# NADOOIT/whisperX

Hardware: AMD Instinct MI355X
Metric: aligned audio-sec/s + word-boundary MAE(ms) vs ref, 1/2/4/8 GPU (higher is better)
Workload: dtype f32; 1 GPU; cfg2: batch=64 x 30 s EN segments, T=1499, V=32, N~U[300,500]; fused HIP align DP (wx_align_dp) on HBM-resident emissions; global_batch=64, seq_len=1499, parallelism=dp1 (per-file sharding, RCCL vocab broadcast)

## Files before the change

### whisperx_amd/csrc/wx_align_dp.h

```cpp
#ifndef WX_ALIGN_DP_H
#define WX_ALIGN_DP_H

#include "wx_dp_config.h"
#include "wx_dp_forward.h"
#include "wx_dp_helpers.h"
#include "wx_dp_prims.h"
#include "wx_dp_tail.h"
#include "wx_dp_timing.h"
#include "wx_dp_walk.h"
#include "wx_wave.h"

namespace wx {

__device__ unsigned split_arrive(uint64_t* c, unsigned epoch, bool lost) {
    uint64_t old = __hip_atomic_load(c, __ATOMIC_RELAXED, __HIP_MEMORY_SCOPE_AGENT);
    while (true) {
        const unsigned cur = ((unsigned)(old >> 32) == epoch) ? (unsigned)old : 0u;
        const unsigned nw = ((cur & 0x7Fu) + 1u) | (cur & 0x80u) | (lost ? 0x80u : 0u);
        const uint64_t nv = ((uint64_t)epoch << 32) | nw;
        if (__hip_atomic_compare_exchange_strong(c, &old, nv, __ATOMIC_RELAXED, __ATOMIC_RELAXED,
                                                 __HIP_MEMORY_SCOPE_AGENT))
            return nw;
    }
}

constexpr int kLatencyLdsFloats = 84 * 1024 / 4;

template <int VS>
struct ColMapLds {
    static constexpr bool kOn = VS == kGatherVS;
    unsigned bm[kOn ? kMaxVocabWords : 1];
    int wpre[kOn ? kMaxVocabWords + 1 : 1];
    int cols[kOn ? kGatherVS : 1];
};

template <int VS>
__device__ __forceinline__ bool prepare_colmap(ColMapLds<VS>& m, ColMap& cm, const int32_t* tok, int N, int blank,
                                               int V) {
    cm.bm = m.bm;
    cm.wpre = m.wpre;
    cm.cols = m.cols;
    cm.n = 0;
    if (!ColMapLds<VS>::kOn) return true;
    cm.n = build_colmap(tok, N, blank, V, m.bm, m.wpre, m.cols);
    return cm.n <= kGatherVS;
}

template <int VS, int W>
constexpr int kCkSlots = (W == 1 || VS == 32) ? 2 * W : W;

constexpr int kSplitWaves = 8;
constexpr int kQ0LdsFrames = 4096;

template <int C, int VS, int W, int H, bool SP = false, int XW = 0>
__device__ __forceinline__ void align_dp_body(const AlignArgs& a) {
    constexpr bool CK = !SP && H == 0 && VS != kGatherVS && W >= 2;
    constexpr bool WT = split_wt<C, VS, SP>();
    constexpr int kLdsFloats = H ? (kLatencyLdsFloats > 4 * kChunk * VS ? kLatencyLdsFloats : 4 * kChunk * VS)
                                 : (CK ? kCkSlots<VS, W> : 2) * kChunk * VS;
    __shared__ float lds[kLdsFloats];
    __shared__ __attribute__((aligned(16))) float c0b[H || (CK && W >= 2) ? 2 * kChunk : 1];
    __shared__ __attribute__((aligned(16))) float xh[W > 1 ? 2 * W * kWave : 1];
    __shared__ unsigned cmask_lds[kMaxLdsFrames / kChunk + 1];
    __shared__ int tsb[3];
    __shared__ int blo_lds;
    __shared__ int colrec_lds[W + H > 1 ? kMaxLdsFrames / kChunk + 1 : 1];
    __shared__ int sbuf_lds[3 * (W + H + XW)];
    __shared__ ColMapLds<VS> cml;
    __shared__ float xg_lds[SP && C == 1 ? 2 * 32 : 1];
    __shared__ float q0_lds[SP && XW > 0 ? kQ0LdsFrames : 1];
    const int P = SP ? a.parts : 1;
    const int part = SP ? ((int)blockIdx.x / kXcdStride) % P : 0;
    const int xslot = (int)blockIdx.x % kXcdStride;
    const int seg = SP ? ((int)blockIdx.x / kXcdStride / P) * kXcdStride +
                             ((a.flags & kArgXcdSpread) ? (xslot - part) & (kXcdStride - 1) : xslot)
                       : (int)blockIdx.x;
    if (SP && seg >= a.S) return;
    const SegDesc d = load_desc(a.em_off, a.tok_off, a.blank_id, seg);
    const int want = (SP || a.parts > 1) ? launch_split_bucket(d.N, a.parts, a.split_id) : bucket_id(d.N, a.mode);
    if (want != (bucket_make(C, W, H ? 1 : 0) | (SP ? kSplitFlag : 0))) return;
    const int lane = (int)threadIdx.x;
    if (d.N <= 0 || d.T <= 0) {
        if (lane == 0 && part == 0) {
            a.t_start[seg] = 0;
            a.status[seg] = 1;
        }
        return;
    }
    ColMap cm;
    const bool slow = !prepare_colmap(cml, cm, a.tok + d.tok0, d.N, d.blank, a.V);
    if (slow && part != 0) return;
    const float* E = a.em + d.row0 * a.V;
    unsigned* bits = a.bits + ((d.row0 >> 5) + seg) * (int64_t)a.bits_stride_cells;
    float* q0 = a.q0 + d.row0;
    float* cn = a.cn + ((d.row0 + kCnPad * (int64_t)seg) & ~(int64_t)3);
    double* c0acc = a.c0acc + ((d.row0 >> 5) + seg);
    WX_STAMP_RT(4);
    WX_STAMP(0);
    Split sp;
    if (SP) {
        sp.p = part;
        sp.P = P;
        sp.lanes = kWave * W * P;
        sp.tag = a.epoch;
        sp.xstride = (kMaxParts - 1) * kHaloCells;
        sp.spin = a.spin;
        uint64_t* xseg = a.xg + ((d.row0 >> 5) + seg) * (int64_t)sp.xstride;
        sp.xin = xseg + (part > 0 ? part - 1 : 0) * kHaloCells;
        sp.xout = xseg + part * kHaloCells;
        sp.xg = xg_lds;
        sp.q0l = (XW > 0 && d.T <= kQ0LdsFrames) ? q0_lds : nullptr;
    }
    if (SP && lane == 0) tsb[2] = 0;
    bool lost = false;
    if (!slow)
        lost = Forward<C, VS, CK ? 2 : 0, W, H != 0, SP, (H > 1 ? 2 : 1)>::run(
            d, E, a.V, a.tok, bits, q0, cn, nullptr, lds, c0b, xh, a.x4 != 0, cm, nullptr, &sp, c0acc);
    WX_STAMP(1);
    if (SP && lost) tsb[2] = 1;
    wait_vm();
    block_fence();
    bool failed = false;
    if (SP && !slow) {
        if (lane == 0) {
            const bool fenced = !WT || (a.flags & kArgFenced);
            if (fenced) {
                __builtin_amdgcn_fence(__ATOMIC_RELEASE, "agent");
                wait_vm();
            }
            const unsigned w = split_arrive(a.arrive + seg, a.epoch, tsb[2] != 0);
            tsb[0] = ((w & 0x7Fu) == (unsigned)P) ? 1 + (int)((w >> 7) & 1u) : 0;
            if (tsb[0]) {
                if (fenced) {
                    __builtin_amdgcn_fence(__ATOMIC_ACQUIRE, "agent");
                    wait_vm();
                }
                __hip_atomic_store(a.arrive + seg, (uint64_t)0, __ATOMIC_RELAXED, __HIP_MEMORY_SCOPE_AGENT);
            }
        }
        __syncthreads();
        if (tsb[0] == 0) {
            WX_STAMP(2);
            WX_STAMP(3);
            WX_STAMP_RT(5);
            return;
        }
        failed = tsb[0] == 2;
        __syncthreads();
    }
    const Layout lay = Layout::make(C, d.N, kWave * W * P);
    if (slow || failed) {
        if (!generic_forward(d.T, d.N, d.blank, E, a.V, a.tok + d.tok0, bits, lay, cn, q0, lds, kLdsFloats)) {
            if (lane == 0) {
                a.t_start[seg] = 0;
                a.status[seg] = slow ? 2 : 3;
            }
            return;
        }
        wait_vm();
        block_fence();
    }
    int32_t* start = a.seg_start + d.tok0;
    WX_T(w0);
    const int nbw = ((d.T - 1) >> 5) + 1;
    const bool lds_walk = d.T <= kMaxLdsFrames;
    const bool q0l_ok = SP && XW > 0 && d.T <= kQ0LdsFrames && !slow && !failed;
    const int K = lds_walk ? max(1, min(W + H + XW, nbw / kSpecMinBlocks)) : 1;
    WX_T(w1);
    WX_TDECL(w2 = 0);
    auto walk_tail = [&](auto& wsrc) {
    int ts = 0, b_lo = -1;
    unsigned* cmask = lds_walk ? cmask_lds : a.cmask + ((d.row0 >> 5) + seg);
    if constexpr (W + H > 1) b_lo = walk_spec(wsrc, d.N, d.T, cn, cmask, lds_walk, K, colrec_lds, sbuf_lds, ts);
    if (lane < kWave) {
        if constexpr (W + H == 1) {
            ts = column_argmax<WT>(cn, d.T);
            b_lo = walk_impl(wsrc, d.N, ts, cmask, lds_walk);
        }
        if (lane == 0) {
            a.t_start[seg] = ts;
            tsb[0] = ts;
        }
        WX_TSET(w2);
        if (!H && b_lo >= 0) {
            wave_fence();
            compact_starts(cmask, b_lo, (ts - 1) >> 5, start);
        }
        if (lane == 0) {
            tsb[1] = b_lo >= 0 ? 1 : 0;
            blo_lds = b_lo;
        }
    } else {
        if (H && !slow && !failed && !q0l_ok) fill_q0(E, a.V, d.T, q0, kWave);
    }
    if constexpr (H != 0) {
        block_fence();
        const int bl = uniform(blo_lds);
        if (bl >= 0) compact_starts_par(cmask, bl, (uniform(tsb[0]) - 1) >> 5, start);
    }
    WX_T(w3);
    WX_TDUMP(lane == 0, 15, w1 - w0, w2 - w1, w3 - w2);
    };
    if constexpr (CK) {
        CkSrc<C, VS> wsrc;
        wsrc.ck = reinterpret_cast<const float*>(bits);
        wsrc.lay = lay;
        wsrc.acc = c0acc;
        wsrc.E = E;
        wsrc.tok = a.tok + d.tok0;
        wsrc.T = d.T;
        wsrc.N = d.N;
        wsrc.V = a.V;
        wsrc.blank = d.blank;
        wsrc.x4 = a.x4 != 0;
        wsrc.slot[0] = lds + uniform((int)threadIdx.x >> 6) * kChunk * VS;
        wsrc.slot[1] = kCkSlots<VS, W> >= 2 * W ? wsrc.slot[0] + W * kChunk * VS : wsrc.slot[0];
        wsrc.junk = xh;
        walk_tail(wsrc);
    } else {
        BitSrc<C, WT> wsrc{bits, lay};
        walk_tail(wsrc);
    }
    wait_vm();
    block_fence();
    const int ts = tsb[0];
    const bool ok = tsb[1] != 0;
    WX_STAMP(2);
    if (lane == 0) a.status[seg] = (ok ? 0 : 1) | (failed ? WX_STATUS_RECOVERED : 0) | (slow ? WX_STATUS_GENERIC : 0);
    if (!ok) return;
    if (d.T + d.N <= kLdsFloats && d.N > 2 * (int)blockDim.x)
        merge_tokens_lds(E, a.V, a.tok + d.tok0, d.N, d.T, ts, q0l_ok ? q0_lds : q0, start, a.seg_end + d.tok0,
                         a.seg_score + d.tok0, lds);
    else
        merge_tokens(E, a.V, a.tok + d.tok0, d.N, ts, q0l_ok ? q0_lds : q0, start, a.seg_end + d.tok0,
                     a.seg_score + d.tok0);
    WX_STAMP(3);
    WX_STAMP_RT(5);
}

template <int C, int VS, int W, int H>
__global__ __launch_bounds__(kWave*(W + H)) __attribute__((amdgpu_waves_per_eu(H || VS == kGatherVS || C > 8 || W == 1 ? 1 : 4, H ? 2 : 8))) void align_dp_kernel(
    AlignArgs a) {
    align_dp_body<C, VS, W, H>(a);
}

template <int C, int VS, int W>
__global__ __launch_bounds__(kWave * kSplitWaves) __attribute__((amdgpu_waves_per_eu(1, 2))) void align_dp_split_kernel(
    AlignArgs a) {
    static_assert(W + 2 <= kSplitWaves && kSplitWaves <= 8, "split workgroup: W DP waves + 2 helpers + walkers");
    align_dp_body<C, VS, W, 2, true, kSplitWaves - W - 2>(a);
}

template <int C, int VS, int W>
__global__ __launch_bounds__(kWave * W) void trellis_kernel(TrellisArgs a) {
    __shared__ float lds[2 * kChunk * VS];
    __shared__ float xh[W > 1 ? 2 * W * kWave : 1];
    __shared__ ColMapLds<VS> cml;
    __shared__ __attribute__((aligned(16))) float rst[W * kWave * C];
    const int seg = blockIdx.x;
    const SegDesc d = load_desc(a.em_off, a.tok_off, a.blank_id, seg);
    if (bucket_id(d.N) != bucket_make(C, W, 0)) return;
    float* tr = a.tr + a.tr_off[seg];
    const int lane = (int)threadIdx.x;
    if (d.N == 0) {
        for (int t = lane; t <= d.T; t += kWave * W) tr[t] = INFINITY;
        return;
    }
    ColMap cm;
    if (!prepare_colmap(cml, cm, a.tok + d.tok0, d.N, d.blank, a.V)) {
        const int64_t n = (int64_t)(d.T + 1) * (d.N + 1);
        for (int64_t i = lane; i < n; i += kWave * W) tr[i] = NAN;
        return;
    }
    const float* E = a.em + d.row0 * a.V;
    Forward<C, VS, 1, W, false>::run(d, E, a.V, a.tok, nullptr, nullptr, nullptr, tr, lds, nullptr, xh, a.x4 != 0,
                                     cm, rst);
}

}

#endif
```

### whisperx_amd/csrc/wx_dp_forward.h

```cpp
#ifndef WX_DP_FORWARD_H
#define WX_DP_FORWARD_H

#include "wx_dp_config.h"
#include "wx_dp_prims.h"
#include "wx_dp_timing.h"
#include "wx_wave.h"

namespace wx {

template <int C>
using cellvec = float __attribute__((ext_vector_type(C)));

template <int VS>
__host__ __device__ constexpr int quad_stride() { return 4 * (VS + 1); }
template <int VS>
__host__ __device__ constexpr int quad_buf_floats() { return 8 * quad_stride<VS>(); }

constexpr int kXSlack = 1;

struct Split {
    int p, P;
    int lanes;
    unsigned tag;
    uint64_t* xin;
    uint64_t* xout;
    int xstride;
    int spin;
    float* xg;
    float* q0l;
};

template <int C, int VS, int MODE, int W, bool H, bool SP = false, int NH = 1>
struct Forward {
    static constexpr int kRowBytes = VS * 4;
    static constexpr int kLanes = kWave * W;
    static constexpr int kBufs = (C == 1 && MODE == 0 && SP && NH == 2 && VS != kGatherVS) ? 5 : (H ? 4 : 2);
    static constexpr bool kPipelined = H || (MODE != 1 && (C <= 6 || (C == 8 && W == 1)));
    static constexpr bool kC0Lds = H || (MODE == 2 && W >= 2);
    using Geo = Geometry<C, (SP ? 2 : W)>;
    static constexpr int kU = kUnroll;
    static_assert(!(H && MODE == 1), "the materialising kernel computes column 0 in wave 0");
    static constexpr bool kReg = C == 1 && MODE == 0 && SP && NH == 2 && VS != kGatherVS;
    static constexpr bool kWT = split_wt<C, VS, SP>();
    static constexpr int kBufFloats = kReg ? quad_buf_floats<VS>() : kChunk * VS;
    static constexpr int kQS = quad_stride<VS>();

    struct State {
        cellvec<C> cur;
        unsigned w[C];
        double acc;
        float col0;
        int t;
        float* rs;
        int jbase;
        int rd[C];
    };

    __device__ __forceinline__ static bool xwait(const uint64_t* xin, int xstride, int q, int l, unsigned tag,
                                                 uint64_t (&xpre)[C], bool& lost, int spin) {
        constexpr int HL = Geometry<C, 2>::HL;
        const unsigned want = tag;
        const uint64_t* gi = xin + (int64_t)q * xstride + min(l, HL - 1) * C;
        bool ok = true;
#pragma unroll
        for (int k = 0; k < C; ++k) ok = ok && (l >= HL || (unsigned)(xpre[k] >> 32) == want);
        const bool first = __all(ok);
        if (!first) {
            for (int it = 0; !lost && !__all(ok) && it < spin; ++it) {
                __builtin_amdgcn_s_sleep(2);
                ok = true;
#pragma unroll
                for (int k = 0; k < C; ++k) {
                    xpre[k] = granule_load(gi + k);
                    ok = ok && (l >= HL || (unsigned)(xpre[k] >> 32) == want);
                }
            }
            __builtin_amdgcn_s_waitcnt(0x0F70);
        }
        lost = lost || !__all(ok);
        return first;
    }

    __device__ __forceinline__ static bool run(const SegDesc& d, const float* __restrict__ E, int V,
                                               const int32_t* __restrict__ tok,
                                               unsigned* __restrict__ bits,
                                               float* __restrict__ q0,
                                               float* __restrict__ cn,
                                               float* __restrict__ tr,
                                               float* lds ,
                                               float* c0b ,
                                               float* xh , bool x4,
                                               const ColMap& cm ,
                                               float* rst = nullptr ,
                                               const Split* sp = nullptr ,
                                               double* c0acc = nullptr ) {
        const int wv = uniform((int)threadIdx.x >> 6);
        const int vw = SP ? sp->p * W + wv : wv;
        const int lanes = SP ? sp->lanes : kLanes;
        const int T = d.T, N = d.N;
        const int nch = (T + kChunk - 1) / kChunk;
        const bool c0prod = MODE == 2 && W >= 2 && wv == 1;
        double c0a = 0.0;
        float c0e = 0.0f;
        const int l0 = lane_id();
        auto c0_load = [&](int qq) { return E[(int64_t)min(qq * kChunk + (l0 & 31), T - 1) * V]; };
        auto c0_make = [&](int qq, float e) {
            float x = l0 >= 32 ? e : 0.0f;
            double a = c0a;
#pragma unroll
            for (int j = 0; j < kChunk; ++j) {
                a += (double)x;
                x = __builtin_bit_cast(float, __builtin_amdgcn_mov_dpp(__builtin_bit_cast(int, x), 0x130 ,
                                                                       0xF, 0xF, true));
            }
            if (l0 == 0) c0acc[qq] = c0a;
            if (l0 < kChunk) c0b[(qq & 1) * kChunk + l0] = col0_value(qq * kChunk + l0, a, T, N);
            c0a = __shfl(a, kChunk);
        };
        if (c0prod && nch > 0) c0_make(0, c0_load(0));
        if (H && wv >= W + NH) {
            float* q0l = SP ? sp->q0l : nullptr;
            const int nxw = (int)(blockDim.x >> 6) - W - NH;
            const int step = kWave * nxw;
            const int l = lane_id();
            int r0 = (wv - W - NH) * kWave;
            float e0 = 0.0f, e1 = 0.0f;
            if (q0l) {
                e0 = E[(int64_t)min(r0 + l, T - 1) * V];
                e1 = E[(int64_t)min(r0 + step + l, T - 1) * V];
            }
            if (kReg) __syncthreads();
            for (int q = 0; q < nch; ++q) {
                __syncthreads();
                if (q0l && r0 < T) {
                    if (r0 + l < T) q0l[r0 + l] = exp_cr(e0);
                    e0 = e1;
                    r0 += step;
                    e1 = E[(int64_t)min(r0 + step + l, T - 1) * V];
                }
            }
            return false;
        }
        if (H && wv >= W) {
            const bool col0 = (!SP || sp->p == 0) && (NH == 1 || wv == W + 1);
            if constexpr (kReg) {
                int t0 = N > 0 ? tok[d.tok0] : 0;
                t0 = (t0 >= 0 && t0 < V) ? t0 : 0;
                return helper_reg(d, E, V, lds, lds + kBufs * kBufFloats, nch, t0, col0, wv == W, x4, sp);
            } else {
                helper(d, E, V, lds, c0b, nch, x4, cm, col0, NH == 1 || wv == W);
            }
            return false;
        }
        const int l = lane_id();
        const Layout L = Layout::make(C, N, lanes);
        if (MODE == 1) {
            if (threadIdx.x == 0) tr[0] = col0_value(0, 0.0, T, N);
            for (int j = (int)threadIdx.x + 1; j <= N; j += kLanes) tr[j] = -INFINITY;
        }
        if ((W > 1 || SP) && vw > 0 && Geo::lane_of(vw, Geo::HL) >= L.G) {
            if (!H && nch > 0) stage_rows<VS, W>(E, V, 0, min(kChunk, T), lds, x4, cm);
            if (kReg) __syncthreads();
            for (int q = 0; q < nch; ++q) {
                wait_vm();
                __syncthreads();
                if (c0prod && q + 1 < nch) c0_make(q + 1, c0_load(q + 1));
                if (!H && q + 1 < nch)
                    stage_rows<VS, W>(E, V, (q + 1) * kChunk, min(kChunk, T - (q + 1) * kChunk),
                                      lds + ((q + 1) % kBufs) * kBufFloats, x4, cm);
            }
            return false;
        }
        const int g = Geo::lane_of(vw, l);
        const bool halo = vw > 0 && l < Geo::HL;
        const bool xpub = SP && wv == W - 1 && sp->p + 1 < sp->P && Geo::lane_of(vw + 1, Geo::HL) < L.G;
        const bool xsub = SP && wv == 0 && sp->p > 0;
        const int f = L.first(g), cnt = L.count(g);
        const bool is_short = g < L.n_short;
        int toff[C];
#pragma unroll
        for (int k = 0; k < C; ++k) {
            const int j = f + k;
            int tk = (k < cnt && j <= N) ? tok[d.tok0 + j - 1] : 0;
            tk = (tk >= 0 && tk < V) ? tk : 0;
            toff[k] = (VS == kGatherVS ? cm.rank(tk) : tk) * 4;
        }
        const int boff = (VS == kGatherVS ? cm.rank(d.blank) : d.blank) * 4;
        int own_w, own_l;
        Geo::owner(L.G - 1, own_w, own_l);
        const bool owner = uniform(own_w) == vw && l == own_l;
        const bool owner_wave = uniform(own_w) == vw;

        State st;
        if (MODE == 1) {
            const int g0 = Geo::lane_of(vw, vw == 0 ? 0 : Geo::HL);
            const int g1 = min(Geo::lane_of(vw, kWave - 1), L.G - 1);
            const int jend = g1 >= g0 ? L.first(g1) + L.count(g1) - 1 : 0;
            st.jbase = g0 < L.G ? L.first(g0) : N + 1;
            const int nown = max(0, jend - st.jbase + 1);
            st.rs = rst + wv * kWave * C;
#pragma unroll
            for (int i = 0; i < C; ++i) {
                const int r = l + kWave * i;
                int gg = 0, kk = 0;
                if (r < nown) L.locate<C>(st.jbase + r - 1, gg, kk);
                st.rd[i] = r < nown ? (gg - Geo::lane_of(vw, 0)) * C + kk : -1;
            }
        }
#pragma unroll
        for (int k = 0; k < C; ++k) st.cur[k] = -INFINITY;
#pragma unroll
        for (int k = 0; k < C; ++k) st.w[k] = 0u;
        st.acc = 0.0;
        st.col0 = col0_value(0, 0.0, T, N);
        st.t = 0;
        const int inf_from = T + 1 - N;

        if (!H && nch > 0) stage_rows<VS, W>(E, V, 0, min(kChunk, T), lds, x4, cm);
        uint64_t xodd[C], xeven[C];
        bool xlost = false;
#pragma unroll
        for (int k = 0; k < C; ++k) xodd[k] = xeven[k] = 0;
        const int xl = min(l, Geo::HL - 1) * C;
        if (SP && xsub && !kReg) {
#pragma unroll
            for (int k = 0; k < C; ++k) {
                xodd[k] = granule_load(sp->xin + (int64_t)min(1, nch - 1) * sp->xstride + xl + k);
                xeven[k] = granule_load(sp->xin + (int64_t)min(2, nch - 1) * sp->xstride + xl + k);
            }
        }
        WX_TDECL(acc_steps = 0, acc_bar = 0, acc_other = 0, x_miss = 0, x_wait = 0, x_slack = 0);
        unsigned wdef[C];
#pragma unroll
        for (int k = 0; k < C; ++k) wdef[k] = 0u;
        auto store_deferred = [&](const int qd) {
#pragma unroll
            for (int k = 0; k < C; ++k) st_pub<kWT>(bits + ((int64_t)qd * C + k) * lanes + g, wdef[k]);
        };
        RegOps opsA, opsB;
        const int etq = (vw == 0 && l == 0) ? VS * 16 : toff[0] * 4;
        const int ebq = boff * 4;
        if (kReg) __syncthreads();
        auto chunk_iter = [&](const int q, uint64_t(&xpre)[C], RegOps& o, RegOps& n, auto own) {
            constexpr bool OWN = decltype(own)::value;
            WX_T(c0);
            float* buf = lds + (q % kBufs) * kBufFloats;
            const int rows = min(kChunk, T - q * kChunk);
            float* xq = xh + (q & 1) * W * kWave;
            if (W > 1 && q > 0 && wv < W - 1 && l >= kWave - Geo::HL) {
#pragma unroll
                for (int k = 0; k < C; ++k) xq[wv * kWave + (l - (kWave - Geo::HL)) * C + k] = st.cur[k];
            }
            if (SP && xpub && q > 0 && l >= kWave - Geo::HL) {
                uint64_t* go = sp->xout + (int64_t)q * sp->xstride + (l - (kWave - Geo::HL)) * C;
#pragma unroll
                for (int k = 0; k < C; ++k) granule_store(go + k, st.cur[k], sp->tag);
            }
            if (SP && xpub) { WX_CQ(q, 1); }
            WX_T(c1);
            if (!H) wait_vm();
            __syncthreads();
            WX_T(c2);
            if (wv == 0) { WX_CQ(q, 0); }
            if (W > 1 && q > 0 && halo && wv > 0) {
#pragma unroll
                for (int k = 0; k < C; ++k) st.cur[k] = xq[(wv - 1) * kWave + l * C + k];
            }
            if (kReg && SP && xsub && q > 0) {
                if (l < Geo::HL) st.cur[0] = sp->xg[(q & 1) * 32 + l];
            } else if (SP && xsub && q > 0) {
                WX_T(x0);
                const bool missed = !xwait(sp->xin, sp->xstride, q, l, sp->tag, xpre, xlost, sp->spin);
                WX_CQ(q, 2);
                if (l < Geo::HL) {
#pragma unroll
                    for (int k = 0; k < C; ++k) st.cur[k] = __builtin_bit_cast(float, (unsigned)xpre[k]);
                }
                WX_T(x1);
                if ((missed || q == 1) && q + kXSlack < nch) {
                    uint64_t tmp[C];
#pragma unroll
                    for (int k = 0; k < C; ++k) tmp[k] = 0;
                    xwait(sp->xin, sp->xstride, q + kXSlack, l, sp->tag, tmp, xlost, sp->spin);
                }
                WX_T(x2);
                WX_TACC(x_miss, missed ? 1 : 0);
                WX_TACC(x_wait, x1 - x0);
                WX_TACC(x_slack, x2 - x1);
                __builtin_amdgcn_sched_barrier(0);
#pragma unroll
                for (int k = 0; k < C; ++k)
                    xpre[k] = granule_load(sp->xin + (int64_t)min(q + 2, nch - 1) * sp->xstride + xl + k);
            }
            if (SP && MODE == 0 && q > 0 && !halo && g < L.G) store_deferred(q - 1);
            if constexpr (MODE == 2) {
                if (!halo && g < L.G) {
                    float* ck = reinterpret_cast<float*>(bits);
#pragma unroll
                    for (int k = 0; k < C; ++k) ck[((int64_t)q * C + k) * lanes + g] = st.cur[k];
                }
                if (!kC0Lds && vw == 0 && l == 0) c0acc[q] = st.acc;
            }
            if (c0prod && q + 1 < nch) c0e = c0_load(q + 1);
            if (!H) {
                if (q + 1 < nch)
                    stage_rows<VS, W>(E, V, (q + 1) * kChunk, min(kChunk, T - (q + 1) * kChunk),
                                      lds + ((q + 1) % kBufs) * kBufFloats, x4, cm);
                if (MODE != 1 && wv == 0 && l < rows) q0[q * kChunk + l] = exp_cr(buf[l * VS]);
            }
            const char* bb = reinterpret_cast<const char*>(buf);
            const float* c0q = kC0Lds ? c0b + (q & 1) * kChunk : nullptr;
            WX_T(c3);
            if constexpr (kReg) {
                if (q == 0) reg_load(o, bb, etq, ebq);
                const char* nb = reinterpret_cast<const char*>(lds + ((q + 1 < nch ? q + 1 : q) % kBufs) * kBufFloats);
                float cur0 = st.cur[0];
                reg_chunk<OWN>(o, n, nb, etq, ebq, cur0, st.w[0], owner, cn, q * kChunk, T);
                st.cur[0] = cur0;
                st.t += rows;
            } else {
                (void)OWN;
                if (vw == 0) {
                    chunk<true>(bb, c0q, rows, toff, boff, st, inf_from, is_short, halo, f, cnt, owner, N, cn, tr);
                } else {
                    chunk<false>(bb, c0q, rows, toff, boff, st, inf_from, is_short, halo, f, cnt, owner, N, cn, tr);
                }
            }
            if (c0prod && q + 1 < nch) c0_make(q + 1, c0e);
            WX_T(c4);
            WX_TACC(acc_steps, c4 - c3);
            WX_TACC(acc_bar, c2 - c1);
            WX_TACC(acc_other, (c1 - c0) + (c3 - c2));
            if (MODE == 0) {
                const int sh = kChunk - rows;
#pragma unroll
                for (int k = 0; k < C; ++k) {
                    const unsigned wq = kReg ? (st.w[k] & (0xFFFFFFFFu << sh))
                                             : ((sh == 0) ? st.w[k] : (st.w[k] << sh));
                    if (SP)
                        wdef[k] = wq;
                    else if (!halo && g < L.G)
                        bits[((int64_t)q * C + k) * lanes + g] = wq;
                    st.w[k] = 0u;
                }
            }
        };
        if constexpr (SP) {
            auto loop = [&](auto own) {
                for (int q = 0; q < nch; q += 2) {
                    chunk_iter(q, xeven, opsA, opsB, own);
                    if (q + 1 < nch) chunk_iter(q + 1, xodd, opsB, opsA, own);
                }
            };
            if (owner_wave)
                loop(BoolTag<true>{});
            else
                loop(BoolTag<false>{});
            if (MODE == 0 && nch > 0 && !halo && g < L.G) store_deferred(nch - 1);
        } else {
            for (int q = 0; q < nch; ++q) chunk_iter(q, xeven, opsA, opsB, BoolTag<true>{});
        }
        WX_TDUMP(l == 0 && MODE != 1, wv, acc_steps, acc_bar, acc_other,
                 if (SP && xsub) { WX_TSTORE(14, x_miss, x_wait, x_slack) });
        return xlost;
    }

    struct RegOps {
        float4 et[kChunk / 4];
        float4 eb[kChunk / 4];
    };
    __device__ __forceinline__ static void reg_load(RegOps& o, const char* buf, int etq, int ebq) {
#pragma unroll
        for (int p = 0; p < kChunk / 4; ++p) {
            o.et[p] = *reinterpret_cast<const float4*>(buf + p * kQS * 4 + etq);
            o.eb[p] = *reinterpret_cast<const float4*>(buf + p * kQS * 4 + ebq);
        }
    }
#define WX_REG_STEP(CUR, NC, ET, EB)                                                                  \
    "v_add_f32 %[s], %[" #CUR "], %[" #EB "]\n\t"                                                   \
    "v_add_f32_dpp %[c], %[" #CUR "], %[" #ET "] wave_shr:1 row_mask:0xf bank_mask:0xf bound_ctrl:1\n\t" \
    "v_cmp_gt_f32 vcc, %[c], %[s]\n\t"                                                              \
    "v_maximum3_f32 %[" #NC "], %[s], %[c], %[c]\n\t"                                               \
    "v_addc_co_u32 %[w], vcc, %[w], %[w], vcc\n\t"
#define WX_REG_OPERANDS                                                                                 \
    : [n0] "=&v"(n[0]), [n1] "=&v"(n[1]), [n2] "=&v"(n[2]), [n3] "=&v"(n[3]), [w] "+v"(w), [s] "=&v"(s),  \
      [c] "=&v"(c)                                                                                          \
    : [cur] "v"(cur), [e0] "v"(et.x), [e1] "v"(et.y), [e2] "v"(et.z), [e3] "v"(et.w), [b0] "v"(eb.x),     \
      [b1] "v"(eb.y), [b2] "v"(eb.z), [b3] "v"(eb.w)                                                         \
    : "vcc"
    template <bool FIRST>
    __device__ __forceinline__ static void reg_steps4(float cur, unsigned& w, const float4& et, const float4& eb,
                                                      float (&n)[4]) {
        float s, c;
        if constexpr (FIRST)
            asm volatile("s_nop 1\n\t" WX_REG_STEP(cur, n0, e0, b0) WX_REG_STEP(n0, n1, e1, b1)
                             WX_REG_STEP(n1, n2, e2, b2) WX_REG_STEP(n2, n3, e3, b3) WX_REG_OPERANDS);
        else
            asm volatile(WX_REG_STEP(cur, n0, e0, b0) WX_REG_STEP(n0, n1, e1, b1) WX_REG_STEP(n1, n2, e2, b2)
                             WX_REG_STEP(n2, n3, e3, b3) WX_REG_OPERANDS);
    }
#undef WX_REG_OPERANDS
#undef WX_REG_STEP
    template <bool OWN>
    __device__ __forceinline__ static void reg_chunk(const RegOps& o, RegOps& n, const char* nb, int etq, int ebq,
                                                     float& cur, unsigned& w, bool owner, float* __restrict__ cn,
                                                     int t0, int T) {
        float hist[OWN ? kChunk : 1];
#pragma unroll
        for (int p = 0; p < kChunk / 4; ++p) {
            n.et[p] = *reinterpret_cast<const float4*>(nb + p * kQS * 4 + etq);
            n.eb[p] = *reinterpret_cast<const float4*>(nb + p * kQS * 4 + ebq);
            __builtin_amdgcn_sched_barrier(0);
            float nv[4];
            if (p == 0)
                reg_steps4<true>(cur, w, o.et[p], o.eb[p], nv);
            else
                reg_steps4<false>(cur, w, o.et[p], o.eb[p], nv);
            if constexpr (OWN) {
#pragma unroll
                for (int j = 0; j < 4; ++j) hist[4 * p + j] = nv[j];
            }
            cur = nv[3];
            __builtin_amdgcn_sched_barrier(0);
        }
        if (OWN && owner) {
#pragma unroll
            for (int i = 0; i < kChunk / 4; ++i)
                st_pub4<kWT>(cn, t0 + 4 * i, make_float4(hist[4 * i], hist[4 * i + 1], hist[4 * i + 2], hist[4 * i + 3]));
        }
    }

    __device__ static void helper(const SegDesc& d, const float* __restrict__ E, int V, float* lds, float* c0b,
                                  int nch, bool x4, const ColMap& cm, bool col0, bool stage = true);
    __device__ __forceinline__ static void column0(int q, int T, int inf_from, const float* buf, float* c0b,
                                                   double& acc);
    __device__ static bool helper_reg(const SegDesc& d, const float* __restrict__ E, int V, float* lds, float* raw,
                                      int nch, int tok0, bool col0, bool stage, bool x4, const Split* sp = nullptr);
    struct C0Rows;
    __device__ static void col0_helper(const SegDesc& d, const float* __restrict__ E, int V, float* lds, int nch,
                                       int tok0);
    static constexpr int kRing = 4;
    static constexpr int kPairs = 8 * VS / kWave;
    __device__ __forceinline__ static void transpose_quads(const float* raw, float* buf);
    struct StgSet;
    __device__ __forceinline__ static void stg_load(StgSet& s, const float* __restrict__ E, int T, int c);
    __device__ __forceinline__ static void stg_write(const StgSet& s, float* buf);
    __device__ static void stager_regs(const SegDesc& d, const float* __restrict__ E, float* lds, int nch);
    __device__ static bool poll_halo(const Split* sp, int q, int nch, bool lost, uint64_t& pre);

    template <bool WAVE0>
    __device__ __forceinline__ static void chunk(const char* bb, const float* c0q, int rows, const int (&toff)[C],
                                                 int boff, State& st, int inf_from, bool is_short, bool halo, int f,
                                                 int cnt, bool owner, int N, float* __restrict__ cn,
                                                 float* __restrict__ tr) {
        constexpr int kColLds = 3, kColFinite = 1, kColAny = 2;
        if (kPipelined && rows == kChunk) {
            if (!WAVE0)
                pipelined_chunk<0>(bb, c0q, toff, boff, st, inf_from, false, halo, f, cnt, owner, N, cn, tr);
            else if (kC0Lds)
                pipelined_chunk<kColLds>(bb, c0q, toff, boff, st, inf_from, is_short, halo, f, cnt, owner, N, cn, tr);
            else if (st.t + kChunk < inf_from)
                pipelined_chunk<kColFinite>(bb, c0q, toff, boff, st, inf_from, is_short, halo, f, cnt, owner, N, cn, tr);
            else
                pipelined_chunk<kColAny>(bb, c0q, toff, boff, st, inf_from, is_short, halo, f, cnt, owner, N, cn, tr);
            return;
        }
        int r = 0;
        for (; r + kU <= rows; r += kU) {
            const char* gb = bb + r * kRowBytes;
            const char* ga[C];
#pragma unroll
            for (int k = 0; k < C; ++k) ga[k] = gb + toff[k];
            float hist[kU];
            if (!WAVE0 || kC0Lds || st.t + kU < inf_from) {
#pragma unroll
                for (int u = 0; u < kU; ++u) {
                    step<!WAVE0 ? 0 : (kC0Lds ? kColLds : kColFinite)>(gb, ga, u * kRowBytes, boff, c0q + r + u, st,
                                                                 inf_from, is_short, halo, f, cnt, N, tr);
                    hist[u] = st.cur[C - 1];
                    ++st.t;
                }
            } else {
#pragma unroll
                for (int u = 0; u < kU; ++u) {
                    step<kColAny>(gb, ga, u * kRowBytes, boff, c0q, st, inf_from, is_short, halo, f, cnt, N, tr);
                    hist[u] = st.cur[C - 1];
                    ++st.t;
                }
            }
            if (MODE != 1 && owner) {
#pragma unroll
                for (int i = 0; i < kU / 4; ++i)
                    st_pub4<kWT>(cn, st.t - kU + 4 * i, make_float4(hist[4 * i], hist[4 * i + 1], hist[4 * i + 2], hist[4 * i + 3]));
            }
        }
        for (; r < rows; ++r) {
            const char* gb = bb + r * kRowBytes;
            const char* ga[C];
#pragma unroll
            for (int k = 0; k < C; ++k) ga[k] = gb + toff[k];
            step<!WAVE0 ? 0 : (kC0Lds ? kColLds : kColAny)>(gb, ga, 0, boff, c0q + r, st, inf_from, is_short, halo, f,
                                                       cnt, N, tr);
            if (MODE != 1 && owner) st_pub<kWT>(cn + st.t, st.cur[C - 1]);
            ++st.t;
        }
    }

    template <int COL>
    __device__ __forceinline__ static void pipelined_chunk(const char* bb, const float* c0q, const int (&toff)[C],
                                                           int boff, State& st, int inf_from, bool is_short,
                                                           bool halo, int f, int cnt, bool owner, int N,
                                                           float* __restrict__ cn, float* __restrict__ tr) {
        const char* ga[C];
#pragma unroll
        for (int k = 0; k < C; ++k) ga[k] = bb + toff[k];
        Row rw[kChunk];
        float c0r[COL == 3 ? kChunk : 1];
        if constexpr (COL == 3) {
#pragma unroll
            for (int i = 0; i < kChunk / 4; ++i) {
                const float4 v = reinterpret_cast<const float4*>(c0q)[i];
                c0r[4 * i] = v.x;
                c0r[4 * i + 1] = v.y;
                c0r[4 * i + 2] = v.z;
                c0r[4 * i + 3] = v.w;
            }
        }
        constexpr int LC = COL == 3 ? 4 : COL;
        auto c0_of = [&](Row& r, int u) {
            if constexpr (COL == 3) r.c0 = c0r[u];
        };
        load_row<LC>(bb, ga, 0, boff, c0q, rw[0]);
        load_row<LC>(bb, ga, kRowBytes, boff, c0q + 1, rw[1]);
        c0_of(rw[0], 0);
        c0_of(rw[1], 1);
        float hist[kUnroll];
#pragma unroll
        for (int u = 0; u < kChunk; ++u) {
            if ((u & 1) == 0 && u + 2 < kChunk) {
                load_row<LC>(bb, ga, (u + 2) * kRowBytes, boff, c0q + u + 2, rw[u + 2]);
                load_row<LC>(bb, ga, (u + 3) * kRowBytes, boff, c0q + u + 3, rw[u + 3]);
                c0_of(rw[u + 2], u + 2);
                c0_of(rw[u + 3], u + 3);
            }
            __builtin_amdgcn_sched_barrier(0);
            advance<COL>(bb, u * kRowBytes, c0q + u, rw[u], st, inf_from, is_short, halo, f, cnt, N, tr);
            hist[u & (kUnroll - 1)] = st.cur[C - 1];
            ++st.t;
            if (MODE != 1 && (u & (kUnroll - 1)) == kUnroll - 1 && owner) {
                st_pub4<kWT>(cn, st.t - kUnroll, make_float4(hist[0], hist[1], hist[2], hist[3]));
                st_pub4<kWT>(cn, st.t - kUnroll + 4, make_float4(hist[4], hist[5], hist[6], hist[7]));
            }
        }
    }

    template <int COL>
    __device__ __forceinline__ static void step(const char* gb, const char* (&ga)[C], int ro, int boff,
                                                const float* c0, State& st, int inf_from, bool is_short, bool halo,
                                                int f, int cnt, int N, float* __restrict__ tr) {
        Row rw;
        load_row<COL>(gb, ga, ro, boff, c0, rw);
        advance<COL>(gb, ro, c0, rw, st, inf_from, is_short, halo, f, cnt, N, tr);
    }

    struct Row {
        float eb;
        float et[C];
        float c0;
    };
    template <int COL>
    __device__ __forceinline__ static void load_row(const char* gb, const char* (&ga)[C], int ro, int boff,
                                                    const float* c0, Row& rw) {
        rw.eb = *reinterpret_cast<const float*>(gb + ro + boff);
#pragma unroll
        for (int k = 0; k < C; ++k) rw.et[k] = *reinterpret_cast<const float*>(ga[k] + ro);
        if (COL == 3) rw.c0 = *c0;
        if (COL == 1 || COL == 2) rw.c0 = *reinterpret_cast<const float*>(gb + ro);
    }

    template <int COL>
    __device__ __forceinline__ static void advance(const char* gb, int ro, const float* c0, const Row& rw, State& st,
                                                   int inf_from, bool is_short, bool halo, int f, int cnt, int N,
                                                   float* __restrict__ tr) {
        const float eb = rw.eb;
        const float(&et)[C] = rw.et;
        const float src = (C > 1 && is_short) ? st.cur[C > 1 ? C - 2 : 0] : st.cur[C - 1];
        float left;
        if (COL) {
            const float c0v = COL == 3 ? rw.c0 : st.col0;
            const float src2 = lane_id() == kWave - 1 ? c0v : src;
            left = __builtin_bit_cast(float, __builtin_amdgcn_mov_dpp(__builtin_bit_cast(int, src2), 0x13C ,
                                                                      0xF, 0xF, true));
        } else {
            left = __builtin_bit_cast(float, __builtin_amdgcn_mov_dpp(__builtin_bit_cast(int, src), 0x138 ,
                                                                      0xF, 0xF, true));
        }
#pragma unroll
        for (int k = C - 1; k >= 0; --k) {
            const float s = st.cur[k] + eb;
            const float c = (k == 0 ? left : st.cur[k > 0 ? k - 1 : 0]) + et[k];
            if (MODE == 0) st.w[k] = shift_in(st.w[k], c, s);
            st.cur[k] = nan_max(s, c);
        }
        if (COL == 1 || COL == 2) {
            const float e0 = rw.c0;
            st.acc += (double)e0;
            st.col0 = (COL == 1 || st.t + 1 < inf_from) ? (float)st.acc : INFINITY;
        }
        if (MODE == 1) {
            float* row = tr + (int64_t)(st.t + 1) * ((int64_t)N + 1);
            if (COL && lane_id() == 0)
                row[0] = COL == 3 ? (st.t + 1 < inf_from ? c0[1] : INFINITY) : st.col0;
            float* rw = st.rs + lane_id() * C;
            if constexpr (C % 4 == 0) {
#pragma unroll
                for (int k = 0; k < C; k += 4)
                    *reinterpret_cast<float4*>(rw + k) = make_float4(st.cur[k], st.cur[k + 1], st.cur[k + 2], st.cur[k + 3]);
            } else if constexpr (C % 2 == 0) {
#pragma unroll
                for (int k = 0; k < C; k += 2) *reinterpret_cast<float2*>(rw + k) = make_float2(st.cur[k], st.cur[k + 1]);
            } else {
#pragma unroll
                for (int k = 0; k < C; ++k) rw[k] = st.cur[k];
            }
            float* own = row + st.jbase + lane_id();
#pragma unroll
            for (int i = 0; i < C; ++i)
                if (st.rd[i] >= 0) own[kWave * i] = st.rs[st.rd[i]];
        }
    }
};

}

#endif
```

Before: 43.49 million audio-sec/s.

## Split register-path forward into dedicated loop with streamlined halo exchange

Moves the register-resident (kReg) forward DP path out of the generic chunk_iter into a dedicated reg_forward routine. It uses precomputed halo read/write pointers with parity double-buffering, defers the owner column stores until after the halo is published, and streamlines bit-word stores, all to shorten the per-chunk critical path between barriers. split_arrive now starts its CAS from a guessed value derived from the part index instead of issuing an initial atomic load. The risks are extra correctness subtlety in the halo pointer arithmetic and CAS retries when the guess is wrong.

```diff
diff --git a/whisperx_amd/csrc/wx_align_dp.h b/whisperx_amd/csrc/wx_align_dp.h
--- a/whisperx_amd/csrc/wx_align_dp.h
+++ b/whisperx_amd/csrc/wx_align_dp.h
@@ -12,8 +12,8 @@
 
 namespace wx {
 
-__device__ unsigned split_arrive(uint64_t* c, unsigned epoch, bool lost) {
-    uint64_t old = __hip_atomic_load(c, __ATOMIC_RELAXED, __HIP_MEMORY_SCOPE_AGENT);
+__device__ unsigned split_arrive(uint64_t* c, unsigned epoch, bool lost, int part) {
+    uint64_t old = part > 0 ? (((uint64_t)epoch << 32) | (unsigned)part) : (uint64_t)0;
     while (true) {
         const unsigned cur = ((unsigned)(old >> 32) == epoch) ? (unsigned)old : 0u;
         const unsigned nw = ((cur & 0x7Fu) + 1u) | (cur & 0x80u) | (lost ? 0x80u : 0u);
@@ -128,7 +128,7 @@
                 __builtin_amdgcn_fence(__ATOMIC_RELEASE, "agent");
                 wait_vm();
             }
-            const unsigned w = split_arrive(a.arrive + seg, a.epoch, tsb[2] != 0);
+            const unsigned w = split_arrive(a.arrive + seg, a.epoch, tsb[2] != 0, part);
             tsb[0] = ((w & 0x7Fu) == (unsigned)P) ? 1 + (int)((w >> 7) & 1u) : 0;
             if (tsb[0]) {
                 if (fenced) {
diff --git a/whisperx_amd/csrc/wx_dp_forward.h b/whisperx_amd/csrc/wx_dp_forward.h
--- a/whisperx_amd/csrc/wx_dp_forward.h
+++ b/whisperx_amd/csrc/wx_dp_forward.h
@@ -190,6 +190,12 @@
         Geo::owner(L.G - 1, own_w, own_l);
         const bool owner = uniform(own_w) == vw && l == own_l;
         const bool owner_wave = uniform(own_w) == vw;
+        if constexpr (kReg) {
+            const int etq = (vw == 0 && l == 0) ? VS * 16 : toff[0] * 4;
+            const int ebq = boff * 4;
+            reg_forward(sp, lds, xh, bits, cn, nch, T, wv, g, L.G, halo, xpub, xsub, owner, owner_wave, etq, ebq);
+            return false;
+        }
 
         State st;
         if (MODE == 1) {
@@ -237,12 +243,7 @@
 #pragma unroll
             for (int k = 0; k < C; ++k) st_pub<kWT>(bits + ((int64_t)qd * C + k) * lanes + g, wdef[k]);
         };
-        RegOps opsA, opsB;
-        const int etq = (vw == 0 && l == 0) ? VS * 16 : toff[0] * 4;
-        const int ebq = boff * 4;
-        if (kReg) __syncthreads();
-        auto chunk_iter = [&](const int q, uint64_t(&xpre)[C], RegOps& o, RegOps& n, auto own) {
-            constexpr bool OWN = decltype(own)::value;
+        auto chunk_iter = [&](const int q, uint64_t(&xpre)[C]) {
             WX_T(c0);
             float* buf = lds + (q % kBufs) * kBufFloats;
             const int rows = min(kChunk, T - q * kChunk);
@@ -266,9 +267,7 @@
 #pragma unroll
                 for (int k = 0; k < C; ++k) st.cur[k] = xq[(wv - 1) * kWave + l * C + k];
             }
-            if (kReg && SP && xsub && q > 0) {
-                if (l < Geo::HL) st.cur[0] = sp->xg[(q & 1) * 32 + l];
-            } else if (SP && xsub && q > 0) {
+            if (SP && xsub && q > 0) {
                 WX_T(x0);
                 const bool missed = !xwait(sp->xin, sp->xstride, q, l, sp->tag, xpre, xlost, sp->spin);
                 WX_CQ(q, 2);
@@ -311,20 +310,10 @@
             const char* bb = reinterpret_cast<const char*>(buf);
             const float* c0q = kC0Lds ? c0b + (q & 1) * kChunk : nullptr;
             WX_T(c3);
-            if constexpr (kReg) {
-                if (q == 0) reg_load(o, bb, etq, ebq);
-                const char* nb = reinterpret_cast<const char*>(lds + ((q + 1 < nch ? q + 1 : q) % kBufs) * kBufFloats);
-                float cur0 = st.cur[0];
-                reg_chunk<OWN>(o, n, nb, etq, ebq, cur0, st.w[0], owner, cn, q * kChunk, T);
-                st.cur[0] = cur0;
-                st.t += rows;
+            if (vw == 0) {
+                chunk<true>(bb, c0q, rows, toff, boff, st, inf_from, is_short, halo, f, cnt, owner, N, cn, tr);
             } else {
-                (void)OWN;
-                if (vw == 0) {
-                    chunk<true>(bb, c0q, rows, toff, boff, st, inf_from, is_short, halo, f, cnt, owner, N, cn, tr);
-                } else {
-                    chunk<false>(bb, c0q, rows, toff, boff, st, inf_from, is_short, halo, f, cnt, owner, N, cn, tr);
-                }
+                chunk<false>(bb, c0q, rows, toff, boff, st, inf_from, is_short, halo, f, cnt, owner, N, cn, tr);
             }
             if (c0prod && q + 1 < nch) c0_make(q + 1, c0e);
             WX_T(c4);
@@ -335,8 +324,7 @@
                 const int sh = kChunk - rows;
 #pragma unroll
                 for (int k = 0; k < C; ++k) {
-                    const unsigned wq = kReg ? (st.w[k] & (0xFFFFFFFFu << sh))
-                                             : ((sh == 0) ? st.w[k] : (st.w[k] << sh));
+                    const unsigned wq = (sh == 0) ? st.w[k] : (st.w[k] << sh);
                     if (SP)
                         wdef[k] = wq;
                     else if (!halo && g < L.G)
@@ -346,19 +334,13 @@
             }
         };
         if constexpr (SP) {
-            auto loop = [&](auto own) {
-                for (int q = 0; q < nch; q += 2) {
-                    chunk_iter(q, xeven, opsA, opsB, own);
-                    if (q + 1 < nch) chunk_iter(q + 1, xodd, opsB, opsA, own);
-                }
-            };
-            if (owner_wave)
-                loop(BoolTag<true>{});
-            else
-                loop(BoolTag<false>{});
+            for (int q = 0; q < nch; q += 2) {
+                chunk_iter(q, xeven);
+                if (q + 1 < nch) chunk_iter(q + 1, xodd);
+            }
             if (MODE == 0 && nch > 0 && !halo && g < L.G) store_deferred(nch - 1);
         } else {
-            for (int q = 0; q < nch; ++q) chunk_iter(q, xeven, opsA, opsB, BoolTag<true>{});
+            for (int q = 0; q < nch; ++q) chunk_iter(q, xeven);
         }
         WX_TDUMP(l == 0 && MODE != 1, wv, acc_steps, acc_bar, acc_other,
                  if (SP && xsub) { WX_TSTORE(14, x_miss, x_wait, x_slack) });
@@ -403,9 +385,7 @@
 #undef WX_REG_STEP
     template <bool OWN>
     __device__ __forceinline__ static void reg_chunk(const RegOps& o, RegOps& n, const char* nb, int etq, int ebq,
-                                                     float& cur, unsigned& w, bool owner, float* __restrict__ cn,
-                                                     int t0, int T) {
-        float hist[OWN ? kChunk : 1];
+                                                     float& cur, unsigned& w, float (&hist)[OWN ? kChunk : 1]) {
 #pragma unroll
         for (int p = 0; p < kChunk / 4; ++p) {
             n.et[p] = *reinterpret_cast<const float4*>(nb + p * kQS * 4 + etq);
@@ -423,11 +403,85 @@
             cur = nv[3];
             __builtin_amdgcn_sched_barrier(0);
         }
-        if (OWN && owner) {
-#pragma unroll
-            for (int i = 0; i < kChunk / 4; ++i)
-                st_pub4<kWT>(cn, t0 + 4 * i, make_float4(hist[4 * i], hist[4 * i + 1], hist[4 * i + 2], hist[4 * i + 3]));
-        }
+    }
+
+    __device__ __forceinline__ static void reg_forward(const Split* sp, float* lds, float* xh,
+                                                       unsigned* __restrict__ bits, float* __restrict__ cn, int nch,
+                                                       int T, int wv, int g, int G, bool halo, bool xpub,
+                                                       bool xsub, bool owner, bool owner_wave, int etq, int ebq) {
+        constexpr int HL = Geo::HL;
+        static_assert(C == 1 && 2 * HL == kWave, "pad slots: a C = 1 halo fills half of a wave's xh row");
+        const int l = lane_id();
+        const int lanes = sp->lanes;
+        constexpr int kBufBytes = kBufFloats * 4;
+        float* const hw = xh + wv * kWave + (l ^ HL);
+        const float* hr[2];
+        hr[0] = (wv > 0 ? xh + (wv - 1) * kWave : (xsub ? sp->xg : xh)) + (l & (HL - 1));
+        hr[1] = hr[0] + ((wv > 0 || !xsub) ? W * kWave : 32);
+        const bool own_word = !halo && g < G;
+        unsigned* wp = bits + ((int64_t)g - lanes);
+        uint64_t* gp = sp->xout + (l - (kWave - HL));
+        int t0 = 0;
+        int rn = kBufBytes;
+        float cur = -INFINITY;
+        unsigned w = 0u, wdef = 0u;
+        RegOps opsA, opsB;
+        WX_TDECL(acc_steps = 0, acc_bar = 0, acc_other = 0);
+        __syncthreads();
+        auto iter = [&](const int q, auto first, auto par, RegOps& o, RegOps& n, auto own) {
+            constexpr bool FIRST = decltype(first)::value, OWN = decltype(own)::value;
+            constexpr int PAR = decltype(par)::value ? 1 : 0;
+            WX_T(c1);
+            __syncthreads();
+            WX_T(c2);
+            if (wv == 0) { WX_CQ(q, 0); }
+            if constexpr (FIRST) {
+                reg_load(o, reinterpret_cast<const char*>(lds), etq, ebq);
+            } else {
+                const float hv = *hr[PAR];
+                cur = halo ? hv : cur;
+                if (own_word) st_pub<kWT>(wp, wdef);
+            }
+            wp += lanes;
+            const char* nb = reinterpret_cast<const char*>(lds) + rn;
+            rn = rn + kBufBytes == kBufs * kBufBytes ? 0 : rn + kBufBytes;
+            WX_T(c3);
+            float hist[OWN ? kChunk : 1];
+            reg_chunk<OWN>(o, n, nb, etq, ebq, cur, w, hist);
+            WX_T(c4);
+            hw[(PAR ^ 1) * W * kWave] = cur;
+            gp += sp->xstride;
+            if (xpub && q + 1 < nch) {
+                if (l >= kWave - HL) granule_store(gp, cur, sp->tag);
+                WX_CQ(q + 1, 1);
+            }
+            __builtin_amdgcn_sched_barrier(0);
+            if (OWN && owner) {
+#pragma unroll
+                for (int i = 0; i < kChunk / 4; ++i)
+                    st_pub4<kWT>(cn, t0 + 4 * i, make_float4(hist[4 * i], hist[4 * i + 1], hist[4 * i + 2], hist[4 * i + 3]));
+            }
+            t0 += kChunk;
+            wdef = w;
+            w = 0u;
+            WX_T(c5);
+            WX_TACC(acc_steps, c4 - c3);
+            WX_TACC(acc_bar, c2 - c1);
+            WX_TACC(acc_other, (c3 - c2) + (c5 - c4));
+        };
+        auto loop = [&](auto own) {
+            if (nch > 0) iter(0, BoolTag<true>{}, BoolTag<false>{}, opsA, opsB, own);
+            for (int q = 1; q < nch; q += 2) {
+                iter(q, BoolTag<false>{}, BoolTag<true>{}, opsB, opsA, own);
+                if (q + 1 < nch) iter(q + 1, BoolTag<false>{}, BoolTag<false>{}, opsA, opsB, own);
+            }
+        };
+        if (owner_wave)
+            loop(BoolTag<true>{});
+        else
+            loop(BoolTag<false>{});
+        if (nch > 0 && own_word) st_pub<kWT>(wp, wdef & (0xFFFFFFFFu << (nch * kChunk - T)));
+        WX_TDUMP(l == 0, wv, acc_steps, acc_bar, acc_other, if (xsub) { WX_TSTORE(14, 0, 0, 0) });
     }
 
     __device__ static void helper(const SegDesc& d, const float* __restrict__ E, int V, float* lds, float* c0b,
```

Result: faster. 45.66 million audio-sec/s (median of 6 runs) (+5.0%).
